# vsergeev/luaradio

Hardware: AMD Instinct MI355X
Metric: MSamples/s per block (128-tap complex FIR headline) + WBFM chain end-to-end (higher is better)
Workload: dtype f32

## Files before the change

### luaradio_amd/csrc/kernels_channelizer.h

```cpp
#pragma once
#include "common.h"
#include "kernels_fir.h"

#ifndef LRHIP_CHAN_EXP
#define LRHIP_CHAN_EXP 0
#endif

namespace lrhip {

#ifndef LRHIP_CHAN_INTERLEAVE
#define LRHIP_CHAN_INTERLEAVE 1
#endif
#ifndef LRHIP_CHAN_RT
#define LRHIP_CHAN_RT 1
#endif
#ifndef LRHIP_CHAN_KSLAB
#define LRHIP_CHAN_KSLAB 32
#endif
constexpr int CHAN_RT = LRHIP_CHAN_RT;
constexpr int CHAN_MT = 64 * CHAN_RT;
constexpr int CHAN_KSLAB = LRHIP_CHAN_KSLAB;

template <int NCT>
__global__ __launch_bounds__(256, CHAN_RT == 1 ? 2 : 1) void channelizer_kernel(const float *__restrict__ hist, const float *__restrict__ x,
                                                             const float *__restrict__ W, float *__restrict__ y,
                                                             int M, long n, long nframes, long first)
{
    constexpr int K2 = 16 * NCT;
    constexpr int K = K2 / 2;
    constexpr int DROW = K2 + 2;
    constexpr int WROW = K2 + 16;
    extern __shared__ __attribute__((aligned(16))) float lds[];
    const int tid = threadIdx.x, lane = tid & 63, wave = tid >> 6;
    const int col = lane & 15, kq = lane >> 4;
    const long f0 = (long)blockIdx.x * CHAN_MT;
    const int nsamp = (CHAN_MT - 1) * K + M;
    const int nflt = 2 * nsamp;
    float *ldsD = lds;
    const int dsize = ((nflt + 2 * (nflt / K2) + 2 + 3) / 4) * 4;
    float *ldsW = lds + dsize;

    const long p0 = first + f0 * K;
    const long xlo = p0 - (M - 1);
    if (xlo >= 0 && xlo + nsamp <= n && ((reinterpret_cast<uintptr_t>(x + 2 * xlo) & 15) == 0)) {
        const float4 *src = reinterpret_cast<const float4 *>(x + 2 * xlo);
        for (int i4 = tid; i4 < nflt / 4; i4 += 256) {
            float4 v = src[i4];
            int a = 4 * i4, p = a + 2 * (a / K2);
            *reinterpret_cast<float2 *>(ldsD + p) = make_float2(v.x, v.y);
            *reinterpret_cast<float2 *>(ldsD + p + 2) = make_float2(v.z, v.w);
        }
        for (int a = (nflt / 4) * 4 + tid; a < nflt; a += 256) ldsD[a + 2 * (a / K2)] = x[2 * xlo + a];
    } else {
        for (int r = tid; r < nsamp; r += 256) {
            int a = 2 * r, p = a + 2 * (a / K2);
            ldsD[p] = stream_at<2>(hist, x, p0 + r, 0, M, n);
            ldsD[p + 1] = stream_at<2>(hist, x, p0 + r, 1, M, n);
        }
    }

    constexpr int SLAB_F4 = CHAN_KSLAB * K2 / 4;
    constexpr int UW = (SLAB_F4 + 255) / 256;
    const float4 *W4 = reinterpret_cast<const float4 *>(W);
    static_assert(UW <= 8, "W slab prefetch: at most 8 float4 per thread");
    float4 w0, w1, w2, w3, w4, w5, w6, w7;
#define LR_CHAN_FOR8(OP) OP(0) OP(1) OP(2) OP(3) OP(4) OP(5) OP(6) OP(7)
#define LR_CHAN_LOAD(U)                                                                          \
    if (U < UW) {                                                                                \
        int i4 = tid + U * 256;                                                                  \
        w##U = W4[wbase + (i4 < SLAB_F4 ? i4 : SLAB_F4 - 1)];                                    \
    }
#define LR_CHAN_PUT(U)                                                                           \
    if (U < UW) {                                                                                \
        int i4 = tid + U * 256;                                                                  \
        if (i4 < SLAB_F4) *reinterpret_cast<float4 *>(wdst + ((4 * i4) / K2) * WROW + (4 * i4) % K2) = w##U; \
    }
    {
        const size_t wbase = 0;
        float *wdst = ldsW;
        LR_CHAN_FOR8(LR_CHAN_LOAD)
        LR_CHAN_FOR8(LR_CHAN_PUT)
    }
    __syncthreads();

    f32x4 acc[CHAN_RT][NCT];
#pragma unroll
    for (int r = 0; r < CHAN_RT; r++)
#pragma unroll
        for (int c = 0; c < NCT; c++) acc[r][c] = (f32x4){0.f, 0.f, 0.f, 0.f};
    const float *abase = ldsD + DROW * (wave * 16 * CHAN_RT + col) + kq;
    const int nslabs = 2 * M / CHAN_KSLAB;
    for (int s = 0; s < nslabs; s++) {
        const float *wcur = ldsW + (s & 1) * (CHAN_KSLAB * WROW);
#if LRHIP_CHAN_EXP == 1
        const bool more = false;
#else
        const bool more = s + 1 < nslabs;
#endif
        if (more) {
            const size_t wbase = (size_t)(s + 1) * SLAB_F4;
            LR_CHAN_FOR8(LR_CHAN_LOAD)
        }
        const float *ap = abase + CHAN_KSLAB * s + 2 * ((CHAN_KSLAB * s) / K2);
        const float *bp = wcur + kq * WROW + col;
        constexpr int NST = CHAN_KSLAB / 4;
        float av[2][CHAN_RT], bv[2][NCT];
        auto fetch = [&](int buf, int st) {
#pragma unroll
            for (int r = 0; r < CHAN_RT; r++) av[buf][r] = ap[16 * r * DROW + 4 * st];
#pragma unroll
            for (int c = 0; c < NCT; c++) bv[buf][c] = bp[4 * st * WROW + 16 * c];
        };
        fetch(0, 0);
#pragma unroll
        for (int st = 0; st < NST; st++) {
#if LRHIP_CHAN_INTERLEAVE
            if (st + 1 < NST) fetch((st + 1) & 1, st + 1);
#pragma unroll
            for (int c = 0; c < NCT; c++)
#pragma unroll
                for (int r = 0; r < CHAN_RT; r++)
                    acc[r][c] = __builtin_amdgcn_mfma_f32_16x16x4f32(av[st & 1][r], bv[st & 1][c], acc[r][c], 0, 0, 0);
#pragma unroll
            for (int i = 0; i < NCT * CHAN_RT; i++) {
                __builtin_amdgcn_sched_group_barrier(0x008, 1, 0);
                __builtin_amdgcn_sched_group_barrier(0x100, 1, 0);
            }
            __builtin_amdgcn_sched_barrier(0);
#else
            if (st + 1 < NST) fetch((st + 1) & 1, st + 1);
            __builtin_amdgcn_sched_barrier(0);
#pragma unroll
            for (int c = 0; c < NCT; c++)
#pragma unroll
                for (int r = 0; r < CHAN_RT; r++)
                    acc[r][c] = __builtin_amdgcn_mfma_f32_16x16x4f32(av[st & 1][r], bv[st & 1][c], acc[r][c], 0, 0, 0);
            __builtin_amdgcn_sched_barrier(0);
#endif
        }
        if (more) {
            float *wdst = ldsW + ((s + 1) & 1) * (CHAN_KSLAB * WROW);
            LR_CHAN_FOR8(LR_CHAN_PUT)
        }
#if LRHIP_CHAN_EXP != 1
        __syncthreads();
#endif
    }

#pragma unroll
    for (int rt = 0; rt < CHAN_RT; rt++)
#pragma unroll
        for (int c = 0; c < NCT; c++)
#pragma unroll
            for (int r = 0; r < 4; r++) {
                long f = f0 + (wave * CHAN_RT + rt) * 16 + 4 * kq + r;
                if (f < nframes) y[f * K2 + 16 * c + col] = acc[rt][c][r];
            }
}

#undef LR_CHAN_FOR8
#undef LR_CHAN_LOAD
#undef LR_CHAN_PUT

}
```

### luaradio_amd/csrc/lrhip.hip

```cpp
#include "../../include/lrhip.h"

#include <cmath>
#include <map>
#include <memory>
#include <string>

#include "common.h"
#include "kernels_elem.h"
#include "kernels_fft.h"
#include "kernels_fir.h"
#include "kernels_firfft.h"
#include "kernels_firdecfft.h"
#include "kernels_firdecim.h"
#include "kernels_channelizer.h"
#include "kernels_pfb.h"
#include "kernels_iir.h"
#include "kernels_agc.h"
#include "kernels_firwin.h"
#include "kernels_firwin2.h"
#include "kernels_firfft4k.h"
#include "kernels_firpols.h"
#include "kernels_firfft64.h"
#include "kernels_interp.h"
#include "kernels_rx.h"
// ... 142 lines not shown
    q->in_size = q->out_size = 4 * q->S;
    q->nb = (int)nb; q->na = (int)na; q->P = (int)na - 1;
    q->seq.nb = (int)nb; q->seq.na = (int)na;
    for (unsigned i = 0; i < nb; i++) q->seq.b[i] = b[i];
    for (unsigned i = 0; i < na; i++) q->seq.a[i] = a[i];
    q->scan = q->P >= 1 && q->P <= IIR_MAX_P && nb <= IIR_MAX_NB;
    if (q->scan) {
        int P = q->P;
        IirCoeffs &co = q->co;
        memset(&co, 0, sizeof(co));
        co.nb = (int)nb; co.P = P;
        for (unsigned i = 0; i < nb; i++) co.b[i] = (float)((double)b[i] / (double)a[0]);
        for (int i = 0; i < P; i++) co.a[i] = (float)((double)a[i + 1] / (double)a[0]);
        std::vector<double> A((size_t)P * P, 0.0), T;
        for (int k = 0; k < P; k++) A[k] = -(double)co.a[k];
        for (int r = 1; r < P; r++) A[r * P + r - 1] = 1.0;
        T = A;
        for (int s = 1; s < IIR_LC; s <<= 1) matmul(T, T, T, P);
        std::vector<float> tpow((size_t)9 * P * P);
        std::vector<double> tpow64((size_t)9 * P * P);
        const double p16 = P == 1 ? T[0] : 0.0;
        for (int k = 0; k <= 8; k++) {
            for (int i = 0; i < P * P; i++) { tpow[(size_t)k * P * P + i] = (float)T[i]; tpow64[(size_t)k * P * P + i] = T[i]; }
            if (k == 8) q->Ttile = T;
            matmul(T, T, T, P);
        }
        if (P == 1 && std::fabs(p16) < 1.0 && p16 != 0.0) {
            const int wc = (int)std::ceil(std::log(1e-12) / std::log(std::fabs(p16)));
            if (wc >= 1 && wc <= 128) q->warm_chunks = wc;
        } else if (P == 1 && p16 == 0.0) {
            q->warm_chunks = 1;
        }
        if (P >= 2 && P <= 4) {
            std::vector<double> A16(tpow64.begin(), tpow64.begin() + P * P), M = A16;
            for (int wc = 1; wc <= 128 && !q->warm_chunks; wc++) {
                double mx = 0.0;
                for (double v : M) mx = std::fabs(v) > mx ? std::fabs(v) : mx;
                if (std::isfinite(mx) && mx < 1e-12) q->warm_chunks = wc;
                matmul(M, A16, M, P);
            }
        }
        if (P == 1) {
            double acc = 1.0;
            for (int l = 0; l < 64; l++) { acc *= p16; tpow.push_back((float)acc); }
        } else if (P <= 4) {
            std::vector<double> A16(tpow64.begin(), tpow64.begin() + P * P), M = A16;
            for (int l = 0; l < 64; l++) {
                for (int i = 0; i < P * P; i++) tpow.push_back((float)M[i]);
                matmul(M, A16, M, P);
            }
        }
        if (P > 4 ? upload(q->d_tpow, tpow64.data(), tpow64.size() * sizeof(double)) : upload(q->d_tpow, tpow.data(), tpow.size() * sizeof(float))) return nullptr;
        if (upload(q->d_ttile, q->Ttile.data(), q->Ttile.size() * sizeof(double))) return nullptr;
        static const bool force_3pass = getenv("LRHIP_IIR_3PASS") != nullptr;
        std::vector<double> W = q->Ttile;
        for (int w = 1; w <= 4 && !force_3pass && !q->warm_tiles; w *= 2) {
            double mx = 0.0;
            bool finite = true;
            for (double v : W) { finite = finite && std::isfinite(v); mx = std::fabs(v) > mx ? std::fabs(v) : mx; }
            if (finite && mx < 1e-46) q->warm_tiles = w;
            matmul(W, W, W, P);
        }
    }
    if (q->reset()) return nullptr;
    return q.release();
}

lrhip_stage_t *lrhip_psd_create(unsigned n, const float *window, double scale, int logarithmic, int input_complex, int fftshift)
{
    if (!(scale > 0.0)) { set_error("psd: scale must be positive"); return nullptr; }
    FftStage *q = fft_build(n);
    if (!q) return nullptr;
    q->in_real = !input_complex;
    q->in_size = input_complex ? 8 : 4;
    q->out_size = 4;
    q->out_kind = logarithmic ? FFT_OUT_PSD_LOG : FFT_OUT_PSD;
    q->out_scale = (float)(1.0 / scale);
    q->shift = fftshift != 0;
    if (window) {
        if (upload(q->window, window, n * sizeof(float))) { delete q; return nullptr; }
        q->has_window = true;
    }
    return q;
}

lrhip_stage_t *lrhip_welch_create(unsigned n, const float *window, double scale, int logarithmic, int input_complex, unsigned overlap)
{
    if (overlap >= n) { set_error("welch: overlap %u must be smaller than the frame length %u", overlap, n); return nullptr; }
    std::unique_ptr<FftStage> psd((FftStage *)lrhip_psd_create(n, window, scale, logarithmic, input_complex, 1));
    if (!psd) return nullptr;
    std::unique_ptr<WelchStage> q(new (std::nothrow) WelchStage());
    if (!q) { set_error("out of memory"); return nullptr; }
    q->N = (int)n; q->hop = (int)(n - overlap);
    q->in_size = input_complex ? 8 : 4; q->out_size = 4;
    q->psd = std::move(psd);
    if (q->reset()) return nullptr;
    return q.release();
}

long lrhip_welch_read(lrhip_stage_t *q, float *avg_host, int reset)
{
    WelchStage *w = q ? dynamic_cast<WelchStage *>(q) : nullptr;
    if (!w) return set_error("welch_read: not a welch stage");
    long frames = w->count;
    if (frames > 0) {
        if (!avg_host) return set_error("null output buffer");
        size_t bytes = (size_t)w->N * sizeof(float);
        if (w->h_avg.reserve(bytes)) return -1;
        LR_HIP(hipMemcpyAsync(w->h_avg.p, w->sum.p, bytes, hipMemcpyDeviceToHost, ctx().stream));
        LR_HIP(hipStreamSynchronize(ctx().stream));
        const float *src = (const float *)w->h_avg.p;
        for (int i = 0; i < w->N; i++) avg_host[i] = src[i] / (float)frames;
    }
    if (reset && w->clear()) return -1;
    return frames;
}

lrhip_stage_t *lrhip_dft_create(unsigned n, int inverse, int real_side)
{
    FftStage *q = fft_build(n);
    if (!q) return nullptr;
    q->inverse = inverse != 0;
    if (!inverse) {
        q->in_real = real_side != 0;
        q->in_size = real_side ? 4 : 8;
        q->out_size = 8;
        q->out_kind = FFT_OUT_COMPLEX;
        q->out_scale = 1.0f;
    } else {
        q->in_real = 0;
        q->in_size = 8;
        q->out_size = real_side ? 4 : 8;
        q->out_kind = real_side ? FFT_OUT_REAL : FFT_OUT_COMPLEX;
        q->out_scale = (float)(1.0 / (double)n);
    }
    return q;
}

lrhip_stage_t *lrhip_format_convert_create(const char *format, int complex_out)
{
    if (!format) { set_error("format: missing format name"); return nullptr; }
    int idx = -1;
    for (size_t i = 0; i < sizeof(kFormats) / sizeof(kFormats[0]); i++)
        if (!strcmp(kFormats[i].name, format)) idx = (int)i;
    if (idx < 0) { set_error("Unsupported format (\"%s\")", format); return nullptr; }
    if (ensure_init()) return nullptr;
    FormatStage *q = new (std::nothrow) FormatStage();
    if (!q) { set_error("out of memory"); return nullptr; }
    q->fmt = idx;
    q->scalars = complex_out ? 2 : 1;
    q->in_size = kFormats[idx].bytes * q->scalars;
    q->out_size = 4 * q->scalars;
    return q;
}

lrhip_stage_t *lrhip_format_pack_create(const char *format, int complex_in)
{
    FormatStage *q = (FormatStage *)lrhip_format_convert_create(format, complex_in);
    if (!q) return nullptr;
    q->pack = true;
    std::swap(q->in_size, q->out_size);
    return q;
}

lrhip_stage_t *lrhip_multiply_constant_create(float re, float im, int constant_complex, int input_complex)
{
    if (constant_complex && !input_complex) { set_error("multiplyconstant: a complex constant takes ComplexFloat32 input only (multiplyconstant.lua:42-44)"); return nullptr; }
    if (ensure_init()) return nullptr;
    MulConstStage *q = new (std::nothrow) MulConstStage();
    if (!q) { set_error("out of memory"); return nullptr; }
    q->cr = re; q->ci = constant_complex ? im : 0.f;
    q->mode = !input_complex ? 0 : (constant_complex ? 2 : 1);
    q->in_size = q->out_size = input_complex ? 8 : 4;
    return q;
}

lrhip_stage_t *lrhip_upsampler_create(unsigned factor, int elem_size)
{
    if (factor < 1) { set_error("upsampler: factor must be >= 1"); return nullptr; }
    if (elem_size != 4 && elem_size != 8) { set_error("upsampler: element size must be 4 or 8"); return nullptr; }
    if (ensure_init()) return nullptr;
    UpsamplerStage *q = new (std::nothrow) UpsamplerStage();
    if (!q) { set_error("out of memory"); return nullptr; }
    q->factor = factor;
    q->in_size = q->out_size = elem_size;
    return q;
}

lrhip_stage_t *lrhip_agc_create(double power_alpha, double gain_alpha, double target, double threshold, int input_complex)
{
    if (!(power_alpha > 0.0 && power_alpha <= 1.0) || !(gain_alpha > 0.0 && gain_alpha <= 1.0)) { set_error("agc: alphas must be in (0, 1]"); return nullptr; }
    if (!(target > 0.0) || !(threshold >= 0.0)) { set_error("agc: target and threshold are linear powers (> 0)"); return nullptr; }
    if (ensure_init()) return nullptr;
    std::unique_ptr<AgcStage> q(new (std::nothrow) AgcStage());
    if (!q) { set_error("out of memory"); return nullptr; }
    q->p = AgcParams{power_alpha, gain_alpha, target, threshold};
    q->S = input_complex ? 2 : 1;
    q->in_size = q->out_size = 4 * q->S;
    if (q->reset()) return nullptr;
    return q.release();
}

lrhip_stage_t *lrhip_powersquelch_create(double alpha, double threshold, int input_complex)
{
    if (!(alpha > 0.0 && alpha <= 1.0)) { set_error("powersquelch: alpha must be in (0, 1]"); return nullptr; }
    AgcStage *q = (AgcStage *)lrhip_agc_create(alpha, 1.0, 1.0, threshold, input_complex);
    if (q) q->squelch = true;
    return q;
}

lrhip_stage_t *lrhip_fmmod_create(double modulation_index)
{
    if (!std::isfinite(modulation_index)) { set_error("fmmod: modulation index must be finite"); return nullptr; }
    if (ensure_init()) return nullptr;
    std::unique_ptr<FmModStage> q(new (std::nothrow) FmModStage());
    if (!q) { set_error("out of memory"); return nullptr; }
    q->k = modulation_index;
    q->in_size = 4; q->out_size = 8;
    if (q->reset()) return nullptr;
    return q.release();
}

lrhip_stage_t *lrhip_unary_create(const char *op, float re, float im, int constant_complex, int input_complex)
{
    if (!op) { set_error("unary: missing operation name"); return nullptr; }
    {
        std::string name;
        std::map<std::string, double> kv;
        const char *c = strchr(op, ':');
        const std::string head(op, c ? (size_t)(c - op) : strlen(op));
        if (head == "preamblesampler") return preamblesampler_create(op);
        if (head == "pam" || head == "qam") return modulator_create(op);
        if (head == "interleave" || head == "deinterleave" || head == "wavpack" || head == "wavunpack") return port_stage_create(op);
        if (head == "pll") return pll_create(op);
        if (head == "rdsframer") return plain_create<RfStage>(op, 8);
        if (head == "scmframer") return plain_create<EfStage<EF_SCM>>(op, EfProto<EF_SCM>::REC);
        if (head == "scmplusframer") return plain_create<EfStage<EF_SCMPLUS>>(op, EfProto<EF_SCMPLUS>::REC);
        if (head == "idmframer") return plain_create<EfStage<EF_IDM>>(op, EfProto<EF_IDM>::REC);
        if (head == "ax25framer") return plain_create<AxStage>(op, AX_REC);
        if (head == "pocsagframer") return plain_create<PgStage>(op, PG_REC);
        if (head == "varicodedecoder") return plain_create<VcStage>(op, 1);
        if (head == "manchesterdecoder") {
            if (!parse_op(op, name, kv, {"invert"})) return nullptr;
            return manchesterdecoder_create(kv, op);
        }
        if (c || digital_unary_op(head)) {
            if (!digital_unary_op(head)) { set_error("unary: unknown operation \"%s\"", op); return nullptr; }
            if (!parse_op(op, name, kv, digital_keys(head))) return nullptr;
            return digital_unary_create(name, kv, op);
        }
    }
    struct { const char *name; int code, in, out; } T[] = {
        {"complexmagnitude", UN_CMAG, 8, 4}, {"complexphase", UN_CPHASE, 8, 4}, {"complextoreal", UN_CREAL, 8, 4},
        {"complextoimag", UN_CIMAG, 8, 4},   {"complexconjugate", UN_CCONJ, 8, 8}, {"realtocomplex", UN_R2C, 4, 8},
        {"absolutevalue", UN_ABS, 4, 4}};
    int code = -1, in = 0, out = 0;
    for (auto &t : T)
        if (!strcmp(t.name, op)) { code = t.code; in = t.in; out = t.out; }
    if (!strcmp(op, "addconstant")) {
        if (constant_complex && !input_complex) { set_error("addconstant: a complex constant takes ComplexFloat32 input only (addconstant.lua:42-44)"); return nullptr; }
        code = !input_complex ? UN_ADDC_REAL : (constant_complex ? UN_ADDC_CPLX : UN_ADDC_CPLX_BY_REAL);
        in = out = input_complex ? 8 : 4;
    }
    if (code < 0) { set_error("unary: unknown operation \"%s\"", op); return nullptr; }
    if (ensure_init()) return nullptr;
    UnaryStage *q = new (std::nothrow) UnaryStage();
    if (!q) { set_error("out of memory"); return nullptr; }
    q->op = code; q->cr = re; q->ci = im;
    q->in_size = in; q->out_size = out;
    return q;
}

lrhip_stage_t *lrhip_delay_create(unsigned num_samples, int elem_size)
{
    if (num_samples < 1) { set_error("Number of samples must be greater than 0"); return nullptr; }
    if (elem_size != 4 && elem_size != 8) { set_error("delay: element size must be 4 or 8"); return nullptr; }
    if (ensure_init()) return nullptr;
    std::unique_ptr<DelayStage> q(new (std::nothrow) DelayStage());
    if (!q) { set_error("out of memory"); return nullptr; }
    q->D = num_samples;
    q->in_size = q->out_size = elem_size;
    if (q->reset()) return nullptr;
    return q.release();
}

lrhip_stage_t *lrhip_hilbert_create(const float *taps, unsigned ntaps)
{
    if (!taps || (ntaps % 2) != 1) { set_error("Number of taps must be odd"); return nullptr; }
    std::unique_ptr<HilbertStage> q(new (std::nothrow) HilbertStage());
    if (!q) { set_error("out of memory"); return nullptr; }
    q->fir.reset(fir_build(taps, ntaps, 0, 0, 1, 0, false, 0.0));
    if (!q->fir) return nullptr;
    q->in_size = 4; q->out_size = 8;
    return q.release();
}

lrhip_stage_t *lrhip_channelizer_create(const float *taps, unsigned ntaps, unsigned nchannels)
{
    if (!taps || ntaps < 32 || (ntaps % 32) != 0 || ntaps > 8192) { set_error("channelizer: ntaps must be a multiple of 32 in [32, 8192]"); return nullptr; }
    if (nchannels != 32 && nchannels != 64) { set_error("channelizer: nchannels must be 32 or 64"); return nullptr; }
    if (ensure_init()) return nullptr;
    std::unique_ptr<ChannelizerStage> q(new (std::nothrow) ChannelizerStage());
    if (!q) { set_error("out of memory"); return nullptr; }
    int M = (int)ntaps, K = (int)nchannels, K2 = 2 * K;
    q->M = M; q->K = K;
    q->in_size = q->out_size = 8;
    std::vector<float> W((size_t)2 * M * K2);
    const double PI2 = 6.283185307179586476925286766559;
    for (int i = 0; i < M; i++)
        for (int c = 0; c < K; c++) {
            int j = M - 1 - i;
            double a = PI2 * (double)(((long)c * j) % K) / K, h = taps[j];
            float gr = (float)(h * std::cos(a)), gi = (float)(h * std::sin(a));
            W[(size_t)(2 * i) * K2 + 2 * c] = gr;
            W[(size_t)(2 * i + 1) * K2 + 2 * c] = -gi;
            W[(size_t)(2 * i) * K2 + 2 * c + 1] = gi;
            W[(size_t)(2 * i + 1) * K2 + 2 * c + 1] = gr;
        }
    if (upload(q->W, W.data(), W.size() * sizeof(float))) return nullptr;
    if (q->reset()) return nullptr;
    return q.release();
}

lrhip_stage_t *lrhip_pfb_channelizer_create(const float *taps, unsigned ntaps, unsigned nchannels)
{
    return lrhip_pfb_oversampled_create(taps, ntaps, nchannels, 1);
}

lrhip_stage_t *lrhip_pfb_oversampled_create(const float *taps, unsigned ntaps, unsigned nchannels, unsigned oversample)
{
    if (const char *why = PfbChannelizerStage::refusal(taps ? ntaps : 0, nchannels, oversample)) { set_error("%s", why); return nullptr; }
    if (ensure_init()) return nullptr;
    std::unique_ptr<PfbChannelizerStage> q(new (std::nothrow) PfbChannelizerStage());
    if (!q) { set_error("out of memory"); return nullptr; }
    const int M = (int)ntaps, K = (int)nchannels;
    q->M = M; q->K = K; q->P = (M + K - 1) / K;
    q->R = (int)oversample; q->D = K / q->R;
    while ((1 << q->log2k) < K) q->log2k++;
    q->in_size = q->out_size = 8;
    std::vector<float> tw((size_t)K);
    for (int m = 0; m < K / 2; m++) {
        double ang = -2.0 * 3.14159265358979323846 * m / K;
        tw[2 * m] = (float)std::cos(ang);
        tw[2 * m + 1] = (float)std::sin(ang);
    }
    if (upload(q->taps, taps, (size_t)M * sizeof(float)) || upload(q->tw, tw.data(), tw.size() * sizeof(float))) return nullptr;
    if (q->reset()) return nullptr;
    return q.release();
}

lrhip_stage_t *lrhip_binary_create(const char *op, int input_complex)
{
    if (!op) { set_error("binary: missing operation name"); return nullptr; }
    if (!strcmp(op, "sampler")) {
        if (ensure_init()) return nullptr;
        std::unique_ptr<SamplerStage> q(new (std::nothrow) SamplerStage());
        if (!q) { set_error("out of memory"); return nullptr; }
        q->in_size = q->out_size = input_complex ? 8 : 4;
        q->in2_size = 4;
        if (q->reset()) return nullptr;
        return q.release();
    }
    int code = !strcmp(op, "multiply") ? BIN_MULTIPLY : !strcmp(op, "multiplyconjugate") ? BIN_MULTIPLY_CONJ
             : !strcmp(op, "add") ? BIN_ADD : !strcmp(op, "subtract") ? BIN_SUBTRACT : !strcmp(op, "floattocomplex") ? BIN_F2C : -1;
    if (code < 0) { set_error("binary: unknown operation \"%s\"", op); return nullptr; }
    if (code == BIN_MULTIPLY_CONJ && !input_complex) { set_error("binary: multiplyconjugate takes ComplexFloat32 inputs (multiplyconjugate.lua:26)"); return nullptr; }
    if (ensure_init()) return nullptr;
    BinaryStage *q = new (std::nothrow) BinaryStage();
    if (!q) { set_error("out of memory"); return nullptr; }
    q->op = code;
    q->in_size = q->out_size = input_complex ? 8 : 4;
    if (code == BIN_F2C) { q->in_size = 4; q->out_size = 8; }
    return q;
}

void lrhip_stage_destroy(lrhip_stage_t *q)
{
    if (!q) return;
    if (ctx().ready) (void)hipStreamSynchronize(ctx().stream);
    delete q;
}

int lrhip_stage_reset(lrhip_stage_t *q) { return q ? q->reset() : set_error("null stage"); }
int lrhip_stage_input_size(const lrhip_stage_t *q) { return q ? q->in_size : set_error("null stage"); }
int lrhip_stage_output_size(const lrhip_stage_t *q) { return q ? q->out_size : set_error("null stage"); }
unsigned long lrhip_stage_max_output(const lrhip_stage_t *q, unsigned long n_in) { return q ? q->max_output(n_in) : 0; }

long lrhip_stage_execute_device(lrhip_stage_t *q, const void *in_dev, unsigned long n_in, void *out_dev, unsigned long out_capacity)
{
    if (!q) return set_error("null stage");
    if (n_in && (!in_dev || (!out_dev && q->max_output(n_in)))) return set_error("null buffer");
    return q->run(in_dev, n_in, out_dev, out_capacity);
}

long lrhip_stage_execute(lrhip_stage_t *q, const void *in_host, unsigned long n_in, void *out_host, unsigned long out_capacity)
{
    if (!q) return set_error("null stage");
    if (dynamic_cast<PortStage *>(q)) return set_error("%s stage takes a port table of device pointers: use lrhip_stage_execute_device", q->kind());
    return host_execute(q->h_in, q->h_out, q->d_in, q->d_out, q->in_size, q->out_size, q->max_output(n_in), in_host, n_in,
                        out_host, out_capacity,
                        [&](const void *di, unsigned long n, void *dout, unsigned long cap) { return q->run(di, n, dout, cap); }, q->align(), q->direct_io_ok());
}

long lrhip_stage_execute2_device(lrhip_stage_t *q, const void *in1_dev, const void *in2_dev, unsigned long n_in, void *out_dev,
                                 unsigned long out_capacity)
{
    if (!q) return set_error("null stage");
    if (n_in && (!in1_dev || !in2_dev || !out_dev)) return set_error("null buffer");
    return q->run2(in1_dev, in2_dev, n_in, out_dev, out_capacity);
}

long lrhip_stage_execute2(lrhip_stage_t *q, const void *in1_host, const void *in2_host, unsigned long n_in, void *out_host,
                          unsigned long out_capacity)
{
    if (!q) return set_error("null stage");
    BinaryStage *b = dynamic_cast<BinaryStage *>(q);
    if (!b) return set_error("%s is not a two-input stage", q->kind());
    if (n_in && !in2_host) return set_error("null input buffer");
    const int in2_size = q->input2_size();
    size_t bytes = (size_t)n_in * in2_size;
    if (b->h_in2.reserve(bytes ? bytes : 16) || b->d_in2.reserve(bytes ? bytes : 16)) return -1;
    if (bytes) {
        memcpy(b->h_in2.p, in2_host, bytes);
        LR_HIP(hipMemcpyAsync(b->d_in2.p, b->h_in2.p, bytes, hipMemcpyHostToDevice, ctx().stream));
    }
    return host_execute(q->h_in, q->h_out, q->d_in, q->d_out, q->in_size, q->out_size, q->max_output(n_in), in1_host, n_in, out_host, out_capacity,
                        [&](const void *di, unsigned long n, void *dout, unsigned long cap) {
                            const size_t first = (size_t)((const char *)di - (const char *)q->d_in.p) / (size_t)q->in_size;
                            return q->run2(di, (const char *)b->d_in2.p + first * (size_t)in2_size, n, dout, cap);
                        });
}

lrhip_chain_t *lrhip_chain_create(lrhip_stage_t **stages, unsigned nstages) { return lrhip_chain_create_ex(stages, nstages, 0u); }

lrhip_chain_t *lrhip_chain_create_ex(lrhip_stage_t **stages, unsigned nstages, unsigned flags)
{
    if (!stages || nstages < 1) { set_error("chain: need at least one stage"); return nullptr; }
    if (flags & ~(unsigned)(LRHIP_CHAIN_EXACT_ROTATOR | LRHIP_CHAIN_NO_POLYPHASE_TAIL | LRHIP_CHAIN_NO_FUSION | LRHIP_CHAIN_NO_SINGLE_LAUNCH)) {
        set_error("chain: unknown flag bits 0x%x", flags);
        return nullptr;
    }
    for (unsigned i = 0; i < nstages; i++)
        if (!stages[i]) { set_error("chain: stage %u is null", i); return nullptr; }
    for (unsigned i = 0; i < nstages; i++)
        if (dynamic_cast<PortStage *>(stages[i])) { set_error("chain: stage %u (%s) takes a port table and cannot be part of a chain", i, stages[i]->kind()); return nullptr; }
    for (unsigned i = 0; i + 1 < nstages; i++)
        if (stages[i]->out_size != stages[i + 1]->in_size) {
            set_error("chain: stage %u (%s) emits %d-byte samples but stage %u (%s) takes %d-byte samples", i, stages[i]->kind(),
                      stages[i]->out_size, i + 1, stages[i + 1]->kind(), stages[i + 1]->in_size);
            return nullptr;
        }
    std::unique_ptr<lrhip_chain> c(new (std::nothrow) lrhip_chain());
    if (!c) { set_error("out of memory"); return nullptr; }
    c->flags = flags;
    const PlanFlags pf{!(flags & LRHIP_CHAIN_NO_FUSION), (flags & LRHIP_CHAIN_EXACT_ROTATOR) != 0, (flags & LRHIP_CHAIN_NO_POLYPHASE_TAIL) != 0,
                       !(flags & LRHIP_CHAIN_NO_SINGLE_LAUNCH)};
    std::vector<lrhip_stage_t *> kept;
    if (pf.fusion && nstages > 1) {
        for (unsigned k = 0; k < nstages; k++) {
            DownsamplerStage *d1 = dynamic_cast<DownsamplerStage *>(stages[k]);
            if (!(d1 && d1->factor == 1)) kept.push_back(stages[k]);
        }
        if (!kept.empty() && kept.size() < nstages) { stages = kept.data(); nstages = (unsigned)kept.size(); }
    }
    Plan plan{stages, nstages, pf, c->ops};
    for (unsigned i = 0; i < nstages;) {
        int used = 0;
        for (size_t r = 0; pf.fusion && !used && r < sizeof kPlanRules / sizeof kPlanRules[0]; r++) used = kPlanRules[r](plan, i);
        if (used < 0) return nullptr;
        if (!used) { c->ops.emplace_back(stages[i]); used = 1; }
        i += (unsigned)used;
    }
    if (pf.fusion) {
        fold_fixups(c->ops);
        if (merge_receivers(c->ops, pf)) return nullptr;
        fold_tuner_records(c->ops);
        if (digital_fuse_tail(c->ops)) return nullptr;
    }
    for (size_t k = 0; k + 1 < c->ops.size(); k++) c->edges.emplace_back(new DeviceBuf());
    return c.release();
}

void lrhip_chain_destroy(lrhip_chain_t *c)
{
    if (!c) return;
    if (ctx().ready) (void)hipStreamSynchronize(ctx().stream);
    delete c;
}

int lrhip_chain_reset(lrhip_chain_t *c)
{
    if (!c) return set_error("null chain");
    if (c->inflight) return set_error("chain reset: %u chunks still in flight", c->inflight);
    c->fill = 0;
    c->discard_in = 0;
    if (ctx().ready) LR_HIP(hipStreamSynchronize(ctx().stream));
    for (auto &o : c->ops)
        if (o.stage->reset()) return -1;
    return 0;
}

unsigned long lrhip_chain_max_output(const lrhip_chain_t *c, unsigned long n_in)
{
    if (!c) return 0;
    unsigned long n = n_in;
    for (auto &o : c->ops) n = o.stage->max_output(n);
    return n;
}

static unsigned long chain_output_bound(const lrhip_chain *c, unsigned long n);

long lrhip_chain_execute_device(lrhip_chain_t *c, const void *in_dev, unsigned long n_in, void *out_dev, unsigned long out_capacity)
{
    if (!c) return set_error("null chain");
    g_launches = 0;
    if (c->discard_in && n_in) {
        const unsigned long k = c->discard_in < n_in ? (unsigned long)c->discard_in : n_in;
        const unsigned long bound = chain_output_bound(c, k);
        if (c->d_discard.reserve((size_t)bound * c->ops.back().stage->out_size + 16)) return -1;
        c->discard_in -= k;
        const unsigned long long left = c->discard_in;
        c->discard_in = 0;
        long rc = lrhip_chain_execute_device(c, in_dev, k, c->d_discard.p, bound);
        c->discard_in = left;
        if (rc < 0) return rc;
        in_dev = (const char *)in_dev + (size_t)k * c->ops.front().stage->in_size;
        n_in -= k;
        if (!n_in) return 0;
    }
    const void *cur = in_dev;
    unsigned long n = n_in;
    for (size_t k = 0; k < c->ops.size(); k++) {
        lrhip_stage *s = c->ops[k].stage;
        bool last = k + 1 == c->ops.size();
        unsigned long need = s->max_output(n);
        void *dst;
        unsigned long cap;
        if (last) {
            dst = out_dev;
            cap = out_capacity;
        } else {
            if (c->edges[k]->reserve((size_t)need * s->out_size + 16)) return -1;
            dst = c->edges[k]->p;
            cap = need;
        }
        long got = s->run(cur, n, dst, cap);
        if (got < 0) return got;
        cur = dst;
        n = (unsigned long)got;
    }
    c->last_launches = g_launches;
    return (long)n;
}

long lrhip_chain_execute(lrhip_chain_t *c, const void *in_host, unsigned long n_in, void *out_host, unsigned long out_capacity)
{
    if (!c) return set_error("null chain");
    return host_execute(c->h_in, c->h_out, c->d_in, c->d_out, c->ops.front().stage->in_size, c->ops.back().stage->out_size,
                        lrhip_chain_max_output(c, n_in), in_host, n_in, out_host, out_capacity,
                        [&](const void *di, unsigned long n, void *dout, unsigned long cap) { return lrhip_chain_execute_device(c, di, n, dout, cap); },
                        lrhip_chain_shard_align(c), c->ops.front().stage->direct_io_ok() && c->ops.back().stage->direct_io_ok());
}

int lrhip_chain_last_launches(const lrhip_chain_t *c) { return c ? c->last_launches : set_error("null chain"); }

int lrhip_chain_in_flight(const lrhip_chain_t *c) { return c ? (int)c->inflight : set_error("null chain"); }

static unsigned long stage_output_bound(const lrhip_stage *s, unsigned long n)
{
    unsigned long m = s->max_output(n);
    if (const FirStage *f = dynamic_cast<const FirStage *>(s))
        if (f->use_fft) m = n + (unsigned long)f->L;
    return (m > n ? m : n) + 64;
}
static unsigned long chain_output_bound(const lrhip_chain *c, unsigned long n)
{
    for (auto &o : c->ops) n = stage_output_bound(o.stage, n);
    return n;
}

int lrhip_chain_set_ring(lrhip_chain_t *c, unsigned depth, unsigned long max_chunk)
{
    if (!c) return set_error("null chain");
    if (depth < 1 || depth > 16) return set_error("ring depth must be 1..16");
    if (max_chunk < 1) return set_error("ring: max_chunk must be >= 1");
    if (c->inflight) return set_error("ring: %u chunks still in flight", c->inflight);
    if (ensure_init()) return -1;
    if (!c->s_in) LR_HIP(hipStreamCreateWithFlags(&c->s_in, hipStreamNonBlocking));
    if (!c->s_out) LR_HIP(hipStreamCreateWithFlags(&c->s_out, hipStreamNonBlocking));
    LR_HIP(hipStreamSynchronize(ctx().stream));
    c->ring.clear();
    int in_size = c->ops.front().stage->in_size, out_size = c->ops.back().stage->out_size;
    unsigned long max_out = chain_output_bound(c, max_chunk);
    for (unsigned i = 0; i < depth; i++) {
        std::unique_ptr<lrhip_chain::Slot> sl(new (std::nothrow) lrhip_chain::Slot());
        if (!sl) return set_error("out of memory");
        if (sl->h_in.reserve((size_t)max_chunk * in_size) || sl->d_in.reserve((size_t)max_chunk * in_size)) return -1;
        if (sl->h_out.reserve((size_t)max_out * out_size) || sl->d_out.reserve((size_t)max_out * out_size)) return -1;
        LR_HIP(hipEventCreateWithFlags(&sl->ev_in, hipEventDisableTiming));
        LR_HIP(hipEventCreateWithFlags(&sl->ev_done, hipEventDisableTiming));
        LR_HIP(hipEventCreateWithFlags(&sl->ev_out, hipEventDisableTiming));
        c->ring.push_back(std::move(sl));
    }
    unsigned long nmax = max_chunk;
    for (size_t k = 0; k + 1 < c->ops.size(); k++) {
        nmax = stage_output_bound(c->ops[k].stage, nmax);
        if (c->edges[k]->reserve((size_t)nmax * c->ops[k].stage->out_size + 16)) return -1;
    }
    c->ring_chunk = max_chunk;
    c->ring_out_cap = max_out;
    c->fill = 0;
    c->head = 0;
    c->inflight = 0;
    return 0;
}

static long chain_submit(lrhip_chain_t *c, const void *in_host, unsigned long n_in, bool allow_inplace);
long lrhip_chain_submit(lrhip_chain_t *c, const void *in_host, unsigned long n_in) { return chain_submit(c, in_host, n_in, true); }
static long chain_submit(lrhip_chain_t *c, const void *in_host, unsigned long n_in, bool allow_inplace)
{
    if (!c) return set_error("null chain");
// ... 553 lines not shown
```

### luaradio_amd/csrc/stage_resample.h

```cpp
#pragma once

struct ResampleStage : lrhip_stage {
    int S = 2, M = 0, L = 1, HQ = 0;
    unsigned long D = 1;
    float c = 1.f;
    DeviceBuf d_taps, d_ttab, hist[2];
    int cur = 0;
    uint64_t Q0 = 0, m0 = 0;
    int interp_J = 0;
    int rat_blocks_per_cu = 0;
    static bool rational_supported(int L, unsigned long D) { return (L == 3 && D == 2) || (L == 2 && D == 3) || (L == 4 && D == 3) || (L == 3 && D == 4) || (L == 5 && D == 4) || (L == 4 && D == 5); }
    int interp_blocks_per_cu = 0;
    static int resample_rounds(long ntiles, long slots)
    {
        static const char *e = getenv("LRHIP_RESAMPLE_ROUNDS");
        if (e) return atoi(e) < 0 ? 0 : atoi(e);
        return ntiles <= slots ? 0 : 1;
    }
    static constexpr int SPAN_MAX = 6144;
    const char *kind() const override { return "resample"; }
    unsigned long max_output(unsigned long n) const override { return (n * (unsigned long)L) / D + 2; }
    int seek(unsigned long long n0, unsigned long long *n0_out) override
    {
        if (reset()) return -1;
        Q0 = n0;
        m0 = (n0 * (uint64_t)L + D - 1) / D;
        *n0_out = m0;
        return 0;
    }
    long memory() const override { return HQ; }
    void rate(unsigned long *num, unsigned long *den) const override { *num = D; *den = (unsigned long)L; }
    static bool fits(int M, int L, unsigned long D) { return L >= 1 && 256 * D / (unsigned long)L + (unsigned long)((M - 1) / L) + 4 <= (unsigned long)SPAN_MAX; }
    int reset() override
    {
        cur = 0; Q0 = 0; m0 = 0;
        size_t hb = (size_t)(HQ > 0 ? HQ : 1) * S * sizeof(float);
        return (zero_fill(hist[0], hb) || zero_fill(hist[1], hb)) ? -1 : 0;
    }
    long run(const void *in_dev, unsigned long n, void *out_dev, unsigned long cap) override
    {
        if (!n) return 0;
        uint64_t hi = (Q0 + n) * (uint64_t)L;
        uint64_t m_end = (hi + D - 1) / D;
        long n_out = (long)(m_end - m0);
        if ((unsigned long)n_out > cap) return set_error("resample: output capacity %lu < %ld", cap, n_out);
        const float *h = (const float *)hist[cur].p;
        float *ho = (float *)hist[cur ^ 1].p;
        if (interp_J > 0 && D == 1 && ((uintptr_t)in_dev & 7) == 0 && ((uintptr_t)out_dev & 7) == 0) {
            auto gi = [&](auto kern, size_t lds_bytes, int tq) -> int {
                if (lds_bytes > 48 * 1024) LR_HIP(hipFuncSetAttribute((const void *)kern, hipFuncAttributeMaxDynamicSharedMemorySize, (int)lds_bytes));
                if (!interp_blocks_per_cu) {
                    int nb = 0;
                    LR_HIP(hipOccupancyMaxActiveBlocksPerMultiprocessor(&nb, kern, FIP_NT, lds_bytes));
                    interp_blocks_per_cu = nb < 1 ? 1 : nb;
                }
                const long ntiles = ((long)n + tq - 1) / tq, slots = (long)ctx().num_cus * interp_blocks_per_cu;
                const int rounds = resample_rounds(ntiles, slots);
                const long wgs = rounds > 0 ? (ntiles + rounds - 1) / rounds : (ntiles < slots ? ntiles : slots);
                hipLaunchKernelGGL(kern, dim3((unsigned)wgs), dim3(FIP_NT), lds_bytes, ctx().stream, h, (const float *)in_dev, (const float *)d_ttab.p,
                                   (float *)out_dev, (long)n, HQ, c, ho, ablation_bits("LRHIP_INTERP_DBG"), rounds);
                return 0;
            };
#define LR_INTERP(LL, JJ) gi(fir_interp_kernel<LL, JJ>, (size_t)FipGeom<LL, JJ>::LDS_FLOATS * sizeof(float), FipGeom<LL, JJ>::TQ)
            int rc = L == 2 ? LR_INTERP(2, 64) : L == 3 ? LR_INTERP(3, 43) : L == 4 ? LR_INTERP(4, 32) : LR_INTERP(5, 26);
#undef LR_INTERP
            if (rc) return rc;
            LR_LAUNCH_CHECK();
            cur ^= 1;
            Q0 += n;
            m0 = m_end;
            return n_out;
        }
        static const bool no_rational = getenv("LRHIP_NO_RATIONAL_WIN") != nullptr;
        if (!no_rational && interp_J > 0 && D > 1 && ((uintptr_t)in_dev & 7) == 0 && ((uintptr_t)out_dev & 7) == 0) {
            auto gr = [&](auto kern, size_t lds_bytes, int tq) -> int {
                if (lds_bytes > 48 * 1024) LR_HIP(hipFuncSetAttribute((const void *)kern, hipFuncAttributeMaxDynamicSharedMemorySize, (int)lds_bytes));
                if (!rat_blocks_per_cu) {
                    int nb = 0;
                    LR_HIP(hipOccupancyMaxActiveBlocksPerMultiprocessor(&nb, kern, 256, lds_bytes));
                    rat_blocks_per_cu = nb < 1 ? 1 : nb;
                }
                const long ntiles = ((long)n + (long)(Q0 % D) + tq - 1) / tq, slots = (long)ctx().num_cus * rat_blocks_per_cu;
                const int rounds = resample_rounds(ntiles, slots);
                const long wgs = rounds > 0 ? (ntiles + rounds - 1) / rounds : (ntiles < slots ? ntiles : slots);
                hipLaunchKernelGGL(kern, dim3((unsigned)wgs), dim3(256), lds_bytes, ctx().stream, h, (const float *)in_dev, (const float *)d_ttab.p,
                                   (float *)out_dev, (long)n, n_out, m0, Q0, HQ, c, ho, rounds);
                return 0;
            };
#define LR_RAT(LL, DD, JJ, RR) gr(fir_rational_kernel<LL, DD, JJ, RR>, (size_t)FrrGeom<LL, DD, JJ, RR>::LDS_FLOATS * sizeof(float), FrrGeom<LL, DD, JJ, RR>::TQ)
            int rc = (L == 3 && D == 2) ? LR_RAT(3, 2, 43, 6) : (L == 2 && D == 3) ? LR_RAT(2, 3, 64, 9) : (L == 4 && D == 3) ? LR_RAT(4, 3, 32, 6)
                   : (L == 3 && D == 4) ? LR_RAT(3, 4, 43, 8) : (L == 5 && D == 4) ? LR_RAT(5, 4, 26, 8) : LR_RAT(4, 5, 32, 10);
#undef LR_RAT
            if (rc) return rc;
            LR_LAUNCH_CHECK();
            cur ^= 1;
            Q0 += n;
            m0 = m_end;
            return n_out;
        }
        int span_cap = (int)(256 * D / (unsigned long)L) + (M - 1) / L + 4;
        size_t lds_bytes = ((size_t)((((M - 1) / L + 1) * L + 3) & ~3) + (size_t)span_cap * S) * sizeof(float);
        auto go = [&](auto kern) -> int {
            if (lds_bytes > 48 * 1024) LR_HIP(hipFuncSetAttribute((const void *)kern, hipFuncAttributeMaxDynamicSharedMemorySize, (int)lds_bytes));
            unsigned grid = n_out > 0 ? (unsigned)((n_out + 255) / 256) : 1;
            hipLaunchKernelGGL(kern, dim3(grid), dim3(256), lds_bytes, ctx().stream, h, (const float *)in_dev, (const float *)d_taps.p, (float *)out_dev, M, L,
                               (long)D, (long)n, n_out, m0, Q0, HQ, c, span_cap, ho);
            return 0;
        };
        int rc = S == 2 ? go(fir_resample_kernel<2>) : go(fir_resample_kernel<1>);
        if (rc) return rc;
        LR_LAUNCH_CHECK();
        cur ^= 1;
        Q0 += n;
        m0 = m_end;
        return n_out;
    }
};

struct ChannelizerStage : lrhip_stage {
    int seek(unsigned long long, unsigned long long *) override { return set_error("seek: not supported by the channelizer stage"); }
    long memory() const override { return -1; }
    int M = 0, K = 0;
    DeviceBuf W, hist[2];
    int cur = 0;
    unsigned long index = 0;
    const char *kind() const override { return "channelizer"; }
    unsigned long max_output(unsigned long n) const override { return (n / K + 1) * K; }
    int reset() override
    {
        cur = 0; index = 0;
        size_t hb = (size_t)(M - 1) * 2 * sizeof(float);
        return (zero_fill(hist[0], hb) || zero_fill(hist[1], hb)) ? -1 : 0;
    }
    template <int NCT>
    int launch(const float *x, long n, float *y, long nframes)
    {
        constexpr int K2 = 16 * NCT;
        int nflt = 2 * ((CHAN_MT - 1) * K + M);
        size_t dsize = (size_t)((nflt + 2 * (nflt / K2) + 2 + 3) / 4) * 4;
        size_t lds_bytes = (dsize + (size_t)2 * CHAN_KSLAB * (K2 + 16)) * sizeof(float);
        auto kern = channelizer_kernel<NCT>;
        if (lds_bytes > 48 * 1024) LR_HIP(hipFuncSetAttribute((const void *)kern, hipFuncAttributeMaxDynamicSharedMemorySize, (int)lds_bytes));
        unsigned grid = (unsigned)((nframes + CHAN_MT - 1) / CHAN_MT);
        hipLaunchKernelGGL(kern, dim3(grid), dim3(256), lds_bytes, ctx().stream, (const float *)hist[cur].p, x, (const float *)W.p, y, M, n,
                           nframes, (long)index);
        LR_LAUNCH_CHECK();
        return 0;
    }
    long run(const void *in_dev, unsigned long n_in, void *out_dev, unsigned long cap) override
    {
        long n = (long)n_in;
        if (n <= 0) return 0;
        long nframes = n_in > index ? (long)((n_in - index + K - 1) / K) : 0;
        if ((unsigned long)(nframes * K) > cap) return set_error("channelizer: output capacity %lu < %ld", cap, nframes * K);
        const float *x = (const float *)in_dev;
        if (nframes > 0) {
            int rc = K == 32 ? launch<4>(x, n, (float *)out_dev, nframes) : launch<8>(x, n, (float *)out_dev, nframes);
            if (rc) return rc;
        }
        unsigned grid = grid_for((unsigned long)(M - 1) * 2, 256);
        hipLaunchKernelGGL(fir_history_kernel<2>, dim3(grid), dim3(256), 0, ctx().stream, (const float *)hist[cur].p, x, (float *)hist[cur ^ 1].p, M, n);
        LR_LAUNCH_CHECK();
        cur ^= 1;
        index = index + (unsigned long)nframes * K - n_in;
        return nframes * K;
    }
};
```

Before: 316,400.

## Channelizer: exploit real taps with split re/im planes and conjugate-symmetric output

Restructures the channelizer GEMM so it multiplies real and imaginary sample planes separately against a real half-size cos/sin coefficient matrix. Each output pair (c, K-c) is then formed from four partial products, which roughly halves the MFMA work and shrinks the weight matrix by a factor of four. The history-copy kernel is folded into block 0 of the channelizer launch, dropping one kernel launch per call, and the K-slab size goes from 32 to 16. The costs are two LDS sample planes instead of one interleaved buffer, strided float2 output stores, and special-case handling of the DC and Nyquist bins.

```diff
diff --git a/luaradio_amd/csrc/kernels_channelizer.h b/luaradio_amd/csrc/kernels_channelizer.h
--- a/luaradio_amd/csrc/kernels_channelizer.h
+++ b/luaradio_amd/csrc/kernels_channelizer.h
@@ -1,164 +1,176 @@
 #pragma once
 #include "common.h"
 #include "kernels_fir.h"
-
-#ifndef LRHIP_CHAN_EXP
-#define LRHIP_CHAN_EXP 0
-#endif
 
 namespace lrhip {
 
 #ifndef LRHIP_CHAN_INTERLEAVE
 #define LRHIP_CHAN_INTERLEAVE 1
 #endif
-#ifndef LRHIP_CHAN_RT
-#define LRHIP_CHAN_RT 1
+#ifndef LRHIP_CHAN_KSLAB
+#define LRHIP_CHAN_KSLAB 16
 #endif
-#ifndef LRHIP_CHAN_KSLAB
-#define LRHIP_CHAN_KSLAB 32
-#endif
-constexpr int CHAN_RT = LRHIP_CHAN_RT;
-constexpr int CHAN_MT = 64 * CHAN_RT;
+constexpr int CHAN_MT = 64;
 constexpr int CHAN_KSLAB = LRHIP_CHAN_KSLAB;
+static_assert(CHAN_KSLAB % 4 == 0 && 32 % CHAN_KSLAB == 0, "a slab is whole k-steps, and divides K and M (both multiples of 32)");
+
+__host__ __device__ constexpr int chan_plane_floats(int M, int K)
+{
+    const int nsamp = (CHAN_MT - 1) * K + M;
+    return ((nsamp + 2 * (nsamp / K) + 2 + 3) / 4) * 4;
+}
+__host__ __device__ constexpr size_t chan_lds_bytes(int M, int K)
+{
+    return ((size_t)2 * chan_plane_floats(M, K) + (size_t)2 * CHAN_KSLAB * (K + 16)) * sizeof(float);
+}
 
 template <int NCT>
-__global__ __launch_bounds__(256, CHAN_RT == 1 ? 2 : 1) void channelizer_kernel(const float *__restrict__ hist, const float *__restrict__ x,
-                                                             const float *__restrict__ W, float *__restrict__ y,
-                                                             int M, long n, long nframes, long first)
+__global__ __launch_bounds__(256, 2) void channelizer_kernel(const float *__restrict__ hist, const float *__restrict__ x,
+                                                             const float *__restrict__ G, float *__restrict__ y,
+                                                             float *__restrict__ hist_out, int M, long n, long nframes, long first)
 {
-    constexpr int K2 = 16 * NCT;
-    constexpr int K = K2 / 2;
-    constexpr int DROW = K2 + 2;
-    constexpr int WROW = K2 + 16;
+    constexpr int K = 16 * NCT;
+    constexpr int H = NCT / 2;
+    constexpr int DROW = K + 2;
+    constexpr int WROW = K + 16;
+    static_assert(NCT % 2 == 0, "gr and gi tiles come in pairs");
     extern __shared__ __attribute__((aligned(16))) float lds[];
     const int tid = threadIdx.x, lane = tid & 63, wave = tid >> 6;
     const int col = lane & 15, kq = lane >> 4;
     const long f0 = (long)blockIdx.x * CHAN_MT;
     const int nsamp = (CHAN_MT - 1) * K + M;
-    const int nflt = 2 * nsamp;
-    float *ldsD = lds;
-    const int dsize = ((nflt + 2 * (nflt / K2) + 2 + 3) / 4) * 4;
-    float *ldsW = lds + dsize;
+    const int psize = chan_plane_floats(M, K);
+    float *ldsRe = lds;
+    float *ldsIm = lds + psize;
+    float *ldsW = lds + 2 * psize;
+
+    if (blockIdx.x == 0)
+        for (int i = tid; i < (M - 1) * 2; i += 256) hist_out[i] = stream_at<2>(hist, x, n + i / 2, i % 2, M, n);
 
     const long p0 = first + f0 * K;
     const long xlo = p0 - (M - 1);
     if (xlo >= 0 && xlo + nsamp <= n && ((reinterpret_cast<uintptr_t>(x + 2 * xlo) & 15) == 0)) {
         const float4 *src = reinterpret_cast<const float4 *>(x + 2 * xlo);
-        for (int i4 = tid; i4 < nflt / 4; i4 += 256) {
+        for (int i4 = tid; i4 < nsamp / 2; i4 += 256) {
             float4 v = src[i4];
-            int a = 4 * i4, p = a + 2 * (a / K2);
-            *reinterpret_cast<float2 *>(ldsD + p) = make_float2(v.x, v.y);
-            *reinterpret_cast<float2 *>(ldsD + p + 2) = make_float2(v.z, v.w);
+            int a = 2 * i4, p = a + 2 * (a / K);
+            *reinterpret_cast<float2 *>(ldsRe + p) = make_float2(v.x, v.z);
+            *reinterpret_cast<float2 *>(ldsIm + p) = make_float2(v.y, v.w);
         }
-        for (int a = (nflt / 4) * 4 + tid; a < nflt; a += 256) ldsD[a + 2 * (a / K2)] = x[2 * xlo + a];
     } else {
         for (int r = tid; r < nsamp; r += 256) {
-            int a = 2 * r, p = a + 2 * (a / K2);
-            ldsD[p] = stream_at<2>(hist, x, p0 + r, 0, M, n);
-            ldsD[p + 1] = stream_at<2>(hist, x, p0 + r, 1, M, n);
+            int p = r + 2 * (r / K);
+            ldsRe[p] = stream_at<2>(hist, x, p0 + r, 0, M, n);
+            ldsIm[p] = stream_at<2>(hist, x, p0 + r, 1, M, n);
         }
     }
 
-    constexpr int SLAB_F4 = CHAN_KSLAB * K2 / 4;
+    constexpr int SLAB_F4 = CHAN_KSLAB * K / 4;
     constexpr int UW = (SLAB_F4 + 255) / 256;
-    const float4 *W4 = reinterpret_cast<const float4 *>(W);
-    static_assert(UW <= 8, "W slab prefetch: at most 8 float4 per thread");
-    float4 w0, w1, w2, w3, w4, w5, w6, w7;
-#define LR_CHAN_FOR8(OP) OP(0) OP(1) OP(2) OP(3) OP(4) OP(5) OP(6) OP(7)
+    const float4 *G4 = reinterpret_cast<const float4 *>(G);
+    static_assert(UW <= 2, "G slab prefetch: at most 2 float4 per thread");
+    float4 w0, w1;
+#define LR_CHAN_FOR2(OP) OP(0) OP(1)
 #define LR_CHAN_LOAD(U)                                                                          \
     if (U < UW) {                                                                                \
         int i4 = tid + U * 256;                                                                  \
-        w##U = W4[wbase + (i4 < SLAB_F4 ? i4 : SLAB_F4 - 1)];                                    \
+        w##U = G4[wbase + (i4 < SLAB_F4 ? i4 : SLAB_F4 - 1)];                                    \
     }
 #define LR_CHAN_PUT(U)                                                                           \
     if (U < UW) {                                                                                \
         int i4 = tid + U * 256;                                                                  \
-        if (i4 < SLAB_F4) *reinterpret_cast<float4 *>(wdst + ((4 * i4) / K2) * WROW + (4 * i4) % K2) = w##U; \
+        if (i4 < SLAB_F4) *reinterpret_cast<float4 *>(wdst + ((4 * i4) / K) * WROW + (4 * i4) % K) = w##U; \
     }
     {
         const size_t wbase = 0;
         float *wdst = ldsW;
-        LR_CHAN_FOR8(LR_CHAN_LOAD)
-        LR_CHAN_FOR8(LR_CHAN_PUT)
+        LR_CHAN_FOR2(LR_CHAN_LOAD)
+        LR_CHAN_FOR2(LR_CHAN_PUT)
     }
     __syncthreads();
 
-    f32x4 acc[CHAN_RT][NCT];
+    f32x4 acc_re[NCT], acc_im[NCT];
 #pragma unroll
-    for (int r = 0; r < CHAN_RT; r++)
-#pragma unroll
-        for (int c = 0; c < NCT; c++) acc[r][c] = (f32x4){0.f, 0.f, 0.f, 0.f};
-    const float *abase = ldsD + DROW * (wave * 16 * CHAN_RT + col) + kq;
-    const int nslabs = 2 * M / CHAN_KSLAB;
+    for (int c = 0; c < NCT; c++) acc_re[c] = acc_im[c] = (f32x4){0.f, 0.f, 0.f, 0.f};
+    const int aoff = DROW * (wave * 16 + col) + kq;
+    const int nslabs = M / CHAN_KSLAB;
     for (int s = 0; s < nslabs; s++) {
         const float *wcur = ldsW + (s & 1) * (CHAN_KSLAB * WROW);
-#if LRHIP_CHAN_EXP == 1
-        const bool more = false;
-#else
         const bool more = s + 1 < nslabs;
-#endif
         if (more) {
             const size_t wbase = (size_t)(s + 1) * SLAB_F4;
-            LR_CHAN_FOR8(LR_CHAN_LOAD)
+            LR_CHAN_FOR2(LR_CHAN_LOAD)
         }
-        const float *ap = abase + CHAN_KSLAB * s + 2 * ((CHAN_KSLAB * s) / K2);
+        const int ao = aoff + CHAN_KSLAB * s + 2 * ((CHAN_KSLAB * s) / K);
+        const float *apr = ldsRe + ao, *api = ldsIm + ao;
         const float *bp = wcur + kq * WROW + col;
         constexpr int NST = CHAN_KSLAB / 4;
-        float av[2][CHAN_RT], bv[2][NCT];
+        float ar[2], ai[2], bv[2][NCT];
         auto fetch = [&](int buf, int st) {
-#pragma unroll
-            for (int r = 0; r < CHAN_RT; r++) av[buf][r] = ap[16 * r * DROW + 4 * st];
+            ar[buf] = apr[4 * st];
+            ai[buf] = api[4 * st];
 #pragma unroll
             for (int c = 0; c < NCT; c++) bv[buf][c] = bp[4 * st * WROW + 16 * c];
+        };
+        auto multiply = [&](int buf) {
+#pragma unroll
+            for (int c = 0; c < NCT; c++) {
+                acc_re[c] = __builtin_amdgcn_mfma_f32_16x16x4f32(ar[buf], bv[buf][c], acc_re[c], 0, 0, 0);
+                acc_im[c] = __builtin_amdgcn_mfma_f32_16x16x4f32(ai[buf], bv[buf][c], acc_im[c], 0, 0, 0);
+            }
         };
         fetch(0, 0);
 #pragma unroll
         for (int st = 0; st < NST; st++) {
+            if (st + 1 < NST) fetch((st + 1) & 1, st + 1);
 #if LRHIP_CHAN_INTERLEAVE
-            if (st + 1 < NST) fetch((st + 1) & 1, st + 1);
+            multiply(st & 1);
 #pragma unroll
-            for (int c = 0; c < NCT; c++)
-#pragma unroll
-                for (int r = 0; r < CHAN_RT; r++)
-                    acc[r][c] = __builtin_amdgcn_mfma_f32_16x16x4f32(av[st & 1][r], bv[st & 1][c], acc[r][c], 0, 0, 0);
-#pragma unroll
-            for (int i = 0; i < NCT * CHAN_RT; i++) {
+            for (int i = 0; i < 2 * NCT; i++) {
                 __builtin_amdgcn_sched_group_barrier(0x008, 1, 0);
                 __builtin_amdgcn_sched_group_barrier(0x100, 1, 0);
             }
             __builtin_amdgcn_sched_barrier(0);
 #else
-            if (st + 1 < NST) fetch((st + 1) & 1, st + 1);
             __builtin_amdgcn_sched_barrier(0);
-#pragma unroll
-            for (int c = 0; c < NCT; c++)
-#pragma unroll
-                for (int r = 0; r < CHAN_RT; r++)
-                    acc[r][c] = __builtin_amdgcn_mfma_f32_16x16x4f32(av[st & 1][r], bv[st & 1][c], acc[r][c], 0, 0, 0);
+            multiply(st & 1);
             __builtin_amdgcn_sched_barrier(0);
 #endif
         }
         if (more) {
             float *wdst = ldsW + ((s + 1) & 1) * (CHAN_KSLAB * WROW);
-            LR_CHAN_FOR8(LR_CHAN_PUT)
+            LR_CHAN_FOR2(LR_CHAN_PUT)
         }
-#if LRHIP_CHAN_EXP != 1
         __syncthreads();
-#endif
     }
 
+    float2 *y2 = reinterpret_cast<float2 *>(y);
 #pragma unroll
-    for (int rt = 0; rt < CHAN_RT; rt++)
+    for (int t = 0; t < H; t++) {
+        const int c = 16 * t + col;
+        const bool real_pair = t == 0 && col == 0;
+        const int cm = real_pair ? K / 2 : K - c;
 #pragma unroll
-        for (int c = 0; c < NCT; c++)
-#pragma unroll
-            for (int r = 0; r < 4; r++) {
-                long f = f0 + (wave * CHAN_RT + rt) * 16 + 4 * kq + r;
-                if (f < nframes) y[f * K2 + 16 * c + col] = acc[rt][c][r];
+        for (int r = 0; r < 4; r++) {
+            const float P1 = acc_re[t][r], P4 = acc_im[t][r], P3 = acc_re[t + H][r], P2 = acc_im[t + H][r];
+            float2 lo, hi;
+            if (real_pair) {
+                lo = make_float2(fmaf(0.0f, P4, P1), fmaf(0.0f, P1, P4));
+                hi = make_float2(fmaf(0.0f, P2, P3), fmaf(0.0f, P3, P2));
+            } else {
+                lo = make_float2(P1 - P2, P3 + P4);
+                hi = make_float2(P1 + P2, P4 - P3);
             }
+            const long f = f0 + wave * 16 + 4 * kq + r;
+            if (f < nframes) {
+                y2[f * K + c] = lo;
+                y2[f * K + cm] = hi;
+            }
+        }
+    }
 }
 
-#undef LR_CHAN_FOR8
+#undef LR_CHAN_FOR2
 #undef LR_CHAN_LOAD
 #undef LR_CHAN_PUT
 
diff --git a/luaradio_amd/csrc/lrhip.hip b/luaradio_amd/csrc/lrhip.hip
--- a/luaradio_amd/csrc/lrhip.hip
+++ b/luaradio_amd/csrc/lrhip.hip
@@ -468,21 +468,20 @@
     if (ensure_init()) return nullptr;
     std::unique_ptr<ChannelizerStage> q(new (std::nothrow) ChannelizerStage());
     if (!q) { set_error("out of memory"); return nullptr; }
-    int M = (int)ntaps, K = (int)nchannels, K2 = 2 * K;
+    int M = (int)ntaps, K = (int)nchannels;
     q->M = M; q->K = K;
     q->in_size = q->out_size = 8;
-    std::vector<float> W((size_t)2 * M * K2);
+    std::vector<float> W((size_t)M * K);
     const double PI2 = 6.283185307179586476925286766559;
-    for (int i = 0; i < M; i++)
-        for (int c = 0; c < K; c++) {
-            int j = M - 1 - i;
-            double a = PI2 * (double)(((long)c * j) % K) / K, h = taps[j];
-            float gr = (float)(h * std::cos(a)), gi = (float)(h * std::sin(a));
-            W[(size_t)(2 * i) * K2 + 2 * c] = gr;
-            W[(size_t)(2 * i + 1) * K2 + 2 * c] = -gi;
-            W[(size_t)(2 * i) * K2 + 2 * c + 1] = gi;
-            W[(size_t)(2 * i + 1) * K2 + 2 * c + 1] = gr;
-        }
+    for (int i = 0; i < M; i++) {
+        int j = M - 1 - i;
+        double h = taps[j];
+        for (int c = 0; c <= K / 2; c++) {
+            double a = PI2 * (double)(((long)c * j) % K) / K;
+            W[(size_t)i * K + (c < K / 2 ? c : K / 2)] = (float)(h * std::cos(a));
+            if (c > 0 && c < K / 2) W[(size_t)i * K + K / 2 + c] = (float)(h * std::sin(a));
+        }
+    }
     if (upload(q->W, W.data(), W.size() * sizeof(float))) return nullptr;
     if (q->reset()) return nullptr;
     return q.release();
diff --git a/luaradio_amd/csrc/stage_resample.h b/luaradio_amd/csrc/stage_resample.h
--- a/luaradio_amd/csrc/stage_resample.h
+++ b/luaradio_amd/csrc/stage_resample.h
@@ -135,15 +135,12 @@
     template <int NCT>
     int launch(const float *x, long n, float *y, long nframes)
     {
-        constexpr int K2 = 16 * NCT;
-        int nflt = 2 * ((CHAN_MT - 1) * K + M);
-        size_t dsize = (size_t)((nflt + 2 * (nflt / K2) + 2 + 3) / 4) * 4;
-        size_t lds_bytes = (dsize + (size_t)2 * CHAN_KSLAB * (K2 + 16)) * sizeof(float);
+        size_t lds_bytes = chan_lds_bytes(M, 16 * NCT);
         auto kern = channelizer_kernel<NCT>;
         if (lds_bytes > 48 * 1024) LR_HIP(hipFuncSetAttribute((const void *)kern, hipFuncAttributeMaxDynamicSharedMemorySize, (int)lds_bytes));
         unsigned grid = (unsigned)((nframes + CHAN_MT - 1) / CHAN_MT);
-        hipLaunchKernelGGL(kern, dim3(grid), dim3(256), lds_bytes, ctx().stream, (const float *)hist[cur].p, x, (const float *)W.p, y, M, n,
-                           nframes, (long)index);
+        hipLaunchKernelGGL(kern, dim3(grid), dim3(256), lds_bytes, ctx().stream, (const float *)hist[cur].p, x, (const float *)W.p, y,
+                           (float *)hist[cur ^ 1].p, M, n, nframes, (long)index);
         LR_LAUNCH_CHECK();
         return 0;
     }
@@ -155,12 +152,13 @@
         if ((unsigned long)(nframes * K) > cap) return set_error("channelizer: output capacity %lu < %ld", cap, nframes * K);
         const float *x = (const float *)in_dev;
         if (nframes > 0) {
-            int rc = K == 32 ? launch<4>(x, n, (float *)out_dev, nframes) : launch<8>(x, n, (float *)out_dev, nframes);
+            int rc = K == 32 ? launch<2>(x, n, (float *)out_dev, nframes) : launch<4>(x, n, (float *)out_dev, nframes);
             if (rc) return rc;
+        } else {
+            unsigned grid = grid_for((unsigned long)(M - 1) * 2, 256);
+            hipLaunchKernelGGL(fir_history_kernel<2>, dim3(grid), dim3(256), 0, ctx().stream, (const float *)hist[cur].p, x, (float *)hist[cur ^ 1].p, M, n);
+            LR_LAUNCH_CHECK();
         }
-        unsigned grid = grid_for((unsigned long)(M - 1) * 2, 256);
-        hipLaunchKernelGGL(fir_history_kernel<2>, dim3(grid), dim3(256), 0, ctx().stream, (const float *)hist[cur].p, x, (float *)hist[cur ^ 1].p, M, n);
-        LR_LAUNCH_CHECK();
         cur ^= 1;
         index = index + (unsigned long)nframes * K - n_in;
         return nframes * K;
```

After: 316,200, median of 2. Within noise of the previous version (-0.1%).
